# ogulcanaydogan/llm-slo-ebpf-toolkit

Hardware: AMD Instinct MI355X
Metric: fault-replay attribution throughput through the agent's BPF-ring -> GPU path (events/s, node-wide); held-out attribution macro-F1 and agent CPU overhead % reported alongside (higher is better)
Workload: dtype fp64 posteriors / fp32 features (exact-int64 time joins)

## Files before the change

### llm_slo_ebpf_toolkit_amd/ops/csrc/agent_bindings.cpp

```cpp
#include <pybind11/numpy.h>
#include <pybind11/pybind11.h>
#include <pybind11/stl.h>

#include <cstring>
#include <memory>
#include <stdexcept>

#include "engine.h"
#include "exemplars.h"
#include "openreq.h"
#include "slisketch.h"

namespace py = pybind11;
using namespace mislo;

namespace {

template <class T>
py::array_t<T> copy_array(const T* p, std::vector<py::ssize_t> shape) {
  py::array_t<T> a(shape);
  size_t n = 1;
  for (auto s : shape) n *= (size_t)s;
  if (n) std::memcpy(a.mutable_data(), p, n * sizeof(T));
  return a;
// ... 583 lines not shown
      .def("results", &PyExemplarTracker::results)
      .def("step_ms", &PyExemplarTracker::step_ms)
      .def("resident", &PyExemplarTracker::resident)
      .def("sync", &PyExemplarTracker::sync)
      .def("close", &PyExemplarTracker::close);
  py::class_<PyEngine>(m, "WindowEngine")
      .def(py::init<int, int, int, int, int, int, int, double, double, int, int, bool, bool, int, float, double, int,
                    int, int, int, int, bool>(),
           py::arg("device") = 0, py::arg("sig_cap") = 1 << 20, py::arg("span_cap") = 16384, py::arg("group_cap") = 64,
           py::arg("user_cap") = 1 << 18, py::arg("n_buffers") = 3, py::arg("max_ahead") = 3,
           py::arg("window_ms") = 2000.0, py::arg("threshold") = 0.7, py::arg("fanout") = 3, py::arg("group_mode") = 1,
           py::arg("use_graphs") = true, py::arg("device_refit") = true, py::arg("n_dom") = 10,
           py::arg("ttft_slo_ms") = 800.0f, py::arg("halo_ms") = 0.0, py::arg("import_cap") = 0,
           py::arg("xchg_cap") = 0, py::arg("shard_rank") = 0, py::arg("shard_world") = 1,
           py::arg("halo_windows") = 3, py::arg("split_rings") = false)
      .def("register_host", &PyEngine::register_host)
      .def("submit", &PyEngine::submit, py::arg("k"), py::arg("kernel"), py::arg("user"), py::arg("spans"),
           py::arg("n_groups"), py::arg("labels") = py::none(), py::arg("bases") = std::vector<int64_t>{},
           py::arg("with_labels") = true, py::arg("learn") = false, py::arg("user_rec") = 64)
      .def("h2d_done", &PyEngine::h2d_done)
      .def("wait_h2d", &PyEngine::wait_h2d)
      .def("query", &PyEngine::query)
      .def("wait", &PyEngine::wait)
      .def("packet", &PyEngine::packet)
      .def("results", &PyEngine::results)
      .def("window_ms", &PyEngine::window_ms)
      .def("copy_ms", [](PyEngine& p, int64_t k) {
        py::gil_scoped_release nogil;
        return p.eng().copy_ms(k);
      })
      .def("set_model_bytes", &PyEngine::set_model_bytes)
      .def("set_app_model", &PyEngine::set_app_model)
      .def("set_p0", &PyEngine::set_p0)
      .def("set_refit", &PyEngine::set_refit, py::arg("alpha") = 2.0, py::arg("prior_pseudo") = 1.0,
           py::arg("inv_temp") = 1.0, py::arg("min_count") = 0.0, py::arg("cap_dom") = -1, py::arg("ceil") = 1.0)
      .def("refit_now", &PyEngine::refit_now)
      .def("set_device_refit", [](PyEngine& p, bool on) { p.eng().set_device_refit(on); })
      .def("score", &PyEngine::score, py::arg("feat"), py::arg("labels") = py::none(), py::arg("app") = py::none())
      .def("set_pods", &PyEngine::set_pods)
      .def("inject_remote", &PyEngine::inject_remote)
      .def("results_all", &PyEngine::results_all)
      .def("set_join_params", &PyEngine::set_join_params)
      .def("init_comm", &PyEngine::init_comm)
      .def("totals", &PyEngine::totals)
      .def("reset_totals", &PyEngine::reset_totals)
      .def("stats_acc", &PyEngine::stats_acc)
      .def("model_bytes", &PyEngine::model_bytes)
      .def("restore", &PyEngine::restore)
      .def("sync", &PyEngine::sync)
      .def("import_state", &PyEngine::import_state)
      .def("sent_block", &PyEngine::sent_block)
      .def("close", &PyEngine::close)
      .def_property_readonly("buffers", &PyEngine::buffers)
      .def_property_readonly("windows_folded", &PyEngine::folded)
      .def_property_readonly("graphs", &PyEngine::graphs)
      .def_property_readonly("host_issue_us", &PyEngine::host_issue_us)
      .def_property_readonly("host_wait_us", &PyEngine::host_wait_us)
      .def_property_readonly("host_dma_issue_us", &PyEngine::host_dma_issue_us)
      .def_property_readonly("host_launch_us", &PyEngine::host_launch_us)
      .def_property_readonly("host_pre_us", [](PyEngine& p) { return p.eng().host_pre_us(); })
      .def_property_readonly("host_dma_split_us", [](PyEngine& p) { return p.eng().host_dma_split_us(); })
      .def_property_readonly("host_tail_us", [](PyEngine& p) { return p.eng().host_tail_us(); })
      .def_property_readonly("has_comm", &PyEngine::has_comm)
      .def_property_readonly("rank", [](PyEngine& p) { return p.eng().rank(); })
      .def_property_readonly("world", [](PyEngine& p) { return p.eng().world(); })
      .def_property_readonly("staged_bytes", &PyEngine::staged_bytes)
      .def_property_readonly("direct_bytes", &PyEngine::direct_bytes);
}
```

### llm_slo_ebpf_toolkit_amd/ops/csrc/engine.h

```cpp
#pragma once

#include <hip/hip_runtime.h>
#include <rccl/rccl.h>

#include <map>
#include <tuple>
#include <type_traits>
#include <vector>

#include "mislo_launch.h"
#include "mislo_packet.h"

namespace mislo {

constexpr uint32_t kCtxRows = 1u << 24;
constexpr uint32_t kPodRows = 1u << 20;
constexpr uint32_t kTraceIdRows = 1u << 24;
constexpr int kHeadBytes = 64;

struct Seg {
  const void* ptr;
  size_t bytes;
};

struct EngineConfig {
  int device = 0;
  int sig_cap = 1 << 20, span_cap = 16384, group_cap = 64;
  int user_cap = 1 << 18;
  int n_buffers = 3, max_ahead = 3;
  double window_ms = 2000.0, threshold = 0.7;
  int fanout = 3, group_mode = 1;
  bool use_graphs = true;
  bool device_refit = true;
  double alpha = 2.0, prior_pseudo = 1.0;
  double inv_temp = 1.0, min_count = 0.0;
  int cap_dom = -1;
  double lik_ceil = 1.0;
  int n_dom = 10;
  float ttft_slo_ms = 800.0f;
  double halo_ms = 0.0;
  int halo_windows = 3;
  int import_cap = 0;
  int xchg_cap = 0;
  int shard_rank = 0, shard_world = 1;
  bool split_rings = false;
};

template <class Byte>
struct ResultViewT {
  template <class T>
  using P = std::conditional_t<std::is_const_v<Byte>, const T, T>*;
  P<double> post;
  P<double> gconf;
  P<float> feat;
  P<int32_t> pred;
  P<uint32_t> evbits;
  P<uint32_t> sli;
  P<uint32_t> app;
  P<uint32_t> late;
};
using ResultView = ResultViewT<const uint8_t>;

struct ResultLayout {
  size_t G;
  size_t gconf() const { return 16 * G * 8; }
  size_t feat() const { return gconf() + G * 8; }
  size_t pred() const { return feat() + 16 * G * 4; }
  size_t evbits() const { return pred() + G * 4; }
  size_t sli() const { return evbits() + 16 * G * 4; }
  size_t bytes() const { return sli() + 6 * G * 4; }
  template <class Byte>
  ResultViewT<Byte> view(Byte* r) const {
    ResultViewT<Byte> v;
    auto set = [r](auto& p, size_t off) { p = reinterpret_cast<std::remove_reference_t<decltype(p)>>(r + off); };
    set(v.post, 0), set(v.gconf, gconf()), set(v.feat, feat()), set(v.pred, pred()), set(v.evbits, evbits());
    set(v.sli, sli()), set(v.app, sli() + 2 * G * 4), set(v.late, sli() + 4 * G * 4);
    return v;
  }
};

struct WindowInput {
  std::vector<Seg> kernel;
  std::vector<Seg> user;
  int user_rec = 64;
  std::vector<Seg> spans;
  int n_groups = 0;
  const int32_t* labels = nullptr;
  int64_t bases[4] = {0, 0, 0, 0};
};

class WindowEngine {
 public:
  explicit WindowEngine(const EngineConfig& cfg);
  ~WindowEngine();
  WindowEngine(const WindowEngine&) = delete;
  WindowEngine& operator=(const WindowEngine&) = delete;

  const EngineConfig& config() const { return cfg_; }
  int buffers() const { return nb_; }

  bool register_host(const void* ptr, size_t bytes);
  void submit(int64_t k, const WindowInput& in, bool with_labels, bool learn);
  bool h2d_done(int64_t k);
  void wait_h2d(int64_t k);
  bool query(int64_t k);
  void wait(int64_t k);
  const double* packet(int64_t k) const { return bufs_[k % nb_].packet_host; }
  ResultView results(int64_t k) const { return layout().view<const uint8_t>(bufs_[k % nb_].res_host); }
  ResultLayout layout() const { return ResultLayout{(size_t)cfg_.group_cap}; }
  std::pair<float, float> window_ms(int64_t k);
  std::vector<float> copy_ms(int64_t k);

  void set_model_bytes(const void* bytes, size_t n);
  void set_refit(double alpha, double prior_pseudo, double inv_temp, double min_count, int cap_dom = -1,
                 double ceil = 1.0);
  void refit_now();
  void set_device_refit(bool on) { cfg_.device_refit = on; }
  void score_features(const float* feat, int n, const int32_t* labels, double* post, int32_t* pred, double* conf,
                      uint32_t* evbits, uint32_t* confusion, const uint32_t* app_cnt = nullptr);
  void set_app_model(const void* bytes, size_t n);
  void set_p0(const double* p0, size_t n);
  void set_pods(const uint32_t* pods, const uint32_t* svcnode, size_t n);
  void inject_remote(const void* blocks, size_t stride, int world, int me);
  void set_join_params(double window_ms, double threshold, int fanout, int group_mode);
  void init_comm(const ncclUniqueId& id, int rank, int world);
  bool has_comm() const { return comm_ != nullptr; }
  int rank() const { return rank_; }
  int world() const { return world_; }
  const uint8_t* results_all(int64_t k) const { return comm_ ? bufs_[k % nb_].res_all_host : bufs_[k % nb_].res_host; }
  size_t result_bytes() const { return layout().bytes(); }

  void totals(double* out);
  void reset_totals();
  void stats_acc(double* out);
  void restore(const double* stats, const void* model, size_t model_bytes, int64_t folded);
  void model_bytes(void* out);
  void sync();
  std::vector<int64_t> import_state();
  std::vector<uint8_t> sent_block();
  int64_t windows_folded() const { return folded_; }
  size_t staged_bytes() const { return staged_bytes_; }
  size_t direct_bytes() const { return direct_bytes_; }
  size_t graphs() const { return graphs_.size(); }
  double host_issue_us() const { return issue_n_ ? issue_us_ / issue_n_ : 0.0; }
  double host_wait_us() const { return issue_n_ ? wait_us_ / issue_n_ : 0.0; }
  double host_dma_issue_us() const { return issue_n_ ? dma_us_ / issue_n_ : 0.0; }
  double host_launch_us() const { return issue_n_ ? launch_us_ / issue_n_ : 0.0; }
  double host_pre_us() const { return issue_n_ ? pre_us_ / issue_n_ : 0.0; }
  double host_tail_us() const { return issue_n_ ? tail_us_ / issue_n_ : 0.0; }

 private:
  int rec_shard_rank() const { return cfg_.split_rings ? 0 : cfg_.shard_rank; }
  int rec_shard_world() const { return cfg_.split_rings ? 1 : cfg_.shard_world; }
  struct Buf;
  enum class Stage : int { Window, Records, Join, XchgSpans, XchgHead, Front, Back };
  static constexpr int kStageSlots = 8;
  void alloc();
// ... 29 lines not shown
  EngineConfig cfg_;
  int nb_, max_ahead_;
  size_t off_kern_ = 0, off_user_ = 0, off_span_ = 0, in_bytes_ = 0;
  size_t kern_bytes() const { return (size_t)kRecStride * (((size_t)cfg_.sig_cap + kBatchSlots - 1) / kBatchSlots); }
  std::vector<std::pair<const uint8_t*, size_t>> registered_;
  size_t staged_bytes_ = 0, direct_bytes_ = 0;
  uint32_t *pod_sn_ = nullptr, *pod_host_ = nullptr;
  unsigned long long* trace_hash_ = nullptr;
  AppModel* app_dev_ = nullptr;
  int n_rows_ = 0;
  int gens_ = 1;
  int slots_ = 1;
  unsigned long long* tmax_ = nullptr;
  KeyTs* g_keys_ = nullptr;
  uint32_t *remote_n_ = nullptr, *sel_cnt_ = nullptr, *sel_off_ = nullptr;
  unsigned long long* sel_mask_ = nullptr;
  int sel_stride_ = 0;
  uint8_t *xsend_ = nullptr, *xrecv_ = nullptr;
  size_t xstride_ = 0, xrecv_bytes_ = 0;
  int nblk_imp_ = 0;
  bool spin_ = false;
  std::vector<uint8_t> inject_;
  size_t inject_stride_ = 0;
  int inject_world_ = 0, inject_me_ = 0;
  int rank_ = 0, world_ = 1;
  hipStream_t side_ = nullptr;
  hipStream_t front_ = nullptr;
  bool overlap_ = false;
  struct BufSet {
    GenMeta* gen;
    int* rows;
    uint32_t *ring_state, *hist, *status, *confusion, *cnt, *gcnt;
    unsigned long long *misc, *dbg, *top3, *gsum;
    double *stats, *stats_count;
    SpanRec* s_rec;
    PartCodes* s_part;
    uint32_t *s_items, *s_part_base, *probe_work;
    PreSpan* s_pre;
  };
  std::vector<BufSet> sets_;
  struct Buf {
    int b;
    uint8_t* in;
    uint8_t* head_host;
    uint8_t* staging;
    double *packet_dev, *packet_host;
    uint8_t *res_dev, *res_host;
    uint8_t *res_all_dev, *res_all_host;
    ResultViewT<uint8_t> res;
    SigRec* imp;
    uint32_t* remote_n;
    const BufSet* set;
    const GenMeta* gen_prev;
    hipEvent_t h2d_done, h2d_part, head_done, front_done, compute_done, comm_done, xchg_done;
    hipEvent_t t_start, t_copy_end, t_comp0, t_comp1, t_end;
    const int* counts() const { return reinterpret_cast<const int*>(in); }
  };
  std::vector<Buf> bufs_;
  hipEvent_t ev_fork_ = nullptr, ev_sigbase_ = nullptr, ev_spans_ = nullptr;
  bool branch_ = false;
  bool xspan_ = false;
  bool exchange() const { return comm_ && cfg_.xchg_cap > 0 && cfg_.import_cap > 0; }
  JoinParams jp_{};
  int nblk_sig_ = 1, nblk_span_ = 1;
  hipStream_t copy_ = nullptr, copy2_ = nullptr, compute_ = nullptr, comm_stream_ = nullptr;
  ncclComm_t comm_ = nullptr;
  ncclComm_t xcomm_ = nullptr;
  uint32_t* ctx_tab_ = nullptr;
  double *totals_ = nullptr, *stats_acc_ = nullptr, *p0_ = nullptr;
  uint8_t* model_dev_ = nullptr;
  std::vector<uint8_t*> model_host_;
  int model_slot_ = 0;
  uint8_t* g_status_ = nullptr;
  PartCodes* g_part_ = nullptr;
  uint32_t *g_part_blk_ = nullptr, *g_part_off_ = nullptr, *g_part_tot_ = nullptr, *g_part_base_ = nullptr,
           *g_items_ = nullptr;
  SigRec* g_rec_ = nullptr;
  uint32_t *s_part_blk_ = nullptr, *s_part_off_ = nullptr, *s_part_tot_ = nullptr;
  float *attrs_ = nullptr, *conf_ = nullptr, *kernel_ms_ = nullptr;
  std::map<std::tuple<int, int, bool, bool>, hipGraphExec_t> graphs_;
  std::vector<bool> warm_;
  std::vector<hipGraph_t> graph_defs_;
  int64_t submitted_ = 0, folded_ = 0;
  double issue_us_ = 0, wait_us_ = 0, dma_us_ = 0, launch_us_ = 0, pre_us_ = 0, tail_us_ = 0;
  double split_us_[4] = {0, 0, 0, 0};

 public:
  std::vector<double> host_dma_split_us() const {
    std::vector<double> v;
    for (double x : split_us_) v.push_back(issue_n_ ? x / issue_n_ : 0.0);
    return v;
  }

 private:
  int64_t issue_n_ = 0;
};

void engine_set_tables(const Tables& t);

}
```

### llm_slo_ebpf_toolkit_amd/ops/csrc/engine.hip

```cpp
#include "engine.h"
#include "mislo_packet_kernels.h"

#include <algorithm>
#include <chrono>
#include <cstdlib>
#include <cmath>
#include <cstring>
#include <stdexcept>
#include <string>

namespace mislo {

namespace {

#define HIPCHECK(x)                                                                                  \
  do {                                                                                               \
    hipError_t _e = (x);                                                                             \
    if (_e != hipSuccess) throw std::runtime_error(std::string("HIP error: ") + hipGetErrorString(_e) + \
                                                   " at " #x);                                       \
  } while (0)

#define NCCLCHECK(x)                                                                                        \
  do {                                                                                                      \
    ncclResult_t _r = (x);                                                                                  \
    if (_r != ncclSuccess) throw std::runtime_error(std::string("RCCL error: ") + ncclGetErrorString(_r) + \
                                                    " at " #x);                                             \
  } while (0)

__global__ void k_accumulate(const double* __restrict__ packet, double* __restrict__ totals, int n,
                             double* __restrict__ host) {
  const int i = blockIdx.x * blockDim.x + threadIdx.x;
  if (i < n) {
    const double v = packet[i];
    totals[i] += v;
    host[i] = v;
  }
}

__global__ __launch_bounds__(256) void k_window_end(const uint32_t* hist, const uint32_t* status,
                                                    const unsigned long long* misc, const unsigned long long* dbg,
                                                    const uint32_t* confusion, const double* stats, const double* count,
                                                    const uint32_t* ring, double* __restrict__ packet,
                                                    double* __restrict__ totals, double* __restrict__ packet_host,
                                                    const uint4* __restrict__ res, uint4* __restrict__ res_host,
                                                    size_t res16) {
  const size_t t = blockIdx.x * (size_t)blockDim.x + threadIdx.x, stride = (size_t)gridDim.x * blockDim.x;
  if (t < (size_t)kPacketLen) {
    const double v = packet_value((int)t, hist, status, misc, dbg, confusion, stats, count, ring);
    packet[t] = v;
    totals[t] += v;
    packet_host[t] = v;
  }
  for (size_t i = t; i < res16; i += stride) res_host[i] = res[i];
}

__global__ void k_to_host(const uint4* __restrict__ src, uint4* __restrict__ dst, size_t n16) {
  for (size_t i = blockIdx.x * (size_t)blockDim.x + threadIdx.x; i < n16; i += (size_t)gridDim.x * blockDim.x)
    dst[i] = src[i];
}

void to_host(const void* src, void* dst, size_t bytes, hipStream_t st) {
  const size_t n16 = (bytes + 15) / 16;
  const int g = (int)std::min<size_t>(64, (n16 + 255) / 256);
  hipLaunchKernelGGL(k_to_host, dim3(g > 0 ? g : 1), dim3(256), 0, st, static_cast<const uint4*>(src),
                     static_cast<uint4*>(dst), n16);
}

constexpr unsigned kEvWait = hipEventDisableTiming | hipEventBlockingSync;

int env_int(const char* name, int unset) {
  const char* v = getenv(name);
  return v ? atoi(v) : unset;
}

struct Lap {
  using clock = std::chrono::steady_clock;
  clock::time_point t = clock::now();
  void operator()(double& acc) {
    const auto n = clock::now();
    acc += std::chrono::duration<double, std::micro>(n - t).count();
    t = n;
  }
};

}

void engine_set_tables(const Tables& t) { set_tables(&t); }

template <class T>
T* WindowEngine::dalloc(size_t n, bool zero) {
  void* p = nullptr;
  HIPCHECK(hipMalloc(&p, n * sizeof(T) + 64));
  own_.dev.push_back(p);
  if (zero) HIPCHECK(hipMemset(p, 0, n * sizeof(T)));
  return static_cast<T*>(p);
}

void* WindowEngine::host_alloc(size_t bytes, unsigned flags) {
  void* h = nullptr;
  HIPCHECK(hipHostMalloc(&h, bytes, flags));
  own_.host.push_back(h);
  return h;
}

void* WindowEngine::host_block(size_t bytes) {
  void* h = host_alloc((bytes + 15) & ~size_t(15), hipHostMallocCoherent | hipHostMallocMapped);
  std::memset(h, 0, bytes);
  return h;
}

hipEvent_t WindowEngine::mk_event(unsigned flags) {
  hipEvent_t e;
  HIPCHECK(hipEventCreateWithFlags(&e, flags));
  own_.events.push_back(e);
  return e;
}

hipStream_t WindowEngine::mk_stream(bool high_priority) {
  hipStream_t s;
  int lo = 0, hi = 0;
  if (high_priority) {
    HIPCHECK(hipDeviceGetStreamPriorityRange(&lo, &hi));
// ... 12 lines not shown
}

WindowEngine::Owner::~Owner() {
  for (hipEvent_t e : events) (void)hipEventDestroy(e);
  for (void* p : host) (void)hipHostFree(p);
  for (void* p : dev) (void)hipFree(p);
  for (hipStream_t s : streams) (void)hipStreamDestroy(s);
}

WindowEngine::WindowEngine(const EngineConfig& cfg) : cfg_(cfg) {
  if (cfg.sig_cap <= 0 || cfg.span_cap <= 0 || cfg.group_cap <= 0 || cfg.group_cap > 4096)
    throw std::invalid_argument("capacities out of range");
  if (cfg.sig_cap >= (1 << 27)) throw std::invalid_argument("sig_cap must be < 2^27 (top-3 key packing)");
  nb_ = std::max(2, cfg.n_buffers);
  max_ahead_ = std::min(nb_, std::max(1, cfg.max_ahead));
  if (cfg.user_cap <= 0 || cfg.user_cap > cfg.sig_cap) throw std::invalid_argument("user_cap must be in [1, sig_cap]");
  if (cfg.import_cap < 0 || cfg.xchg_cap < 0 || cfg.halo_ms < 0) throw std::invalid_argument("negative import sizes");
  if (cfg.halo_windows < 1 || cfg.halo_windows >= kMaxGens)
    throw std::invalid_argument("halo_windows must be in [1, 3] (resident generations)");
  gens_ = cfg.halo_ms > 0 ? 1 + cfg.halo_windows : 1;
  if (2LL * gens_ * ((long long)cfg.sig_cap + cfg.import_cap) >= (1LL << 27))
    throw std::invalid_argument("2 x generations x (sig_cap + import_cap) must be < 2^27 (top-3 key packing)");
  HIPCHECK(hipSetDevice(cfg.device));
  set_join_params(cfg.window_ms, cfg.threshold, cfg.fanout, cfg.group_mode);
  alloc();
}

void WindowEngine::set_join_params(double window_ms, double threshold, int fanout, int group_mode) {
  const int64_t ms = 1000000;
  int64_t outer = (int64_t)llround(window_ms * ms);
  if (outer <= 0) outer = 2000 * ms;
  if (outer >= (1LL << 35)) throw std::invalid_argument("window too large for top-3 key packing (< 34 s)");
  jp_.outer_ns = outer;
  const int64_t tw[4] = {outer, 100 * ms, 250 * ms, 500 * ms};
  for (int k = 0; k < 4; ++k) jp_.win_ns[k] = std::min(outer, tw[k]);
  const float cf[4] = {1.0f, 0.9f, 0.8f, 0.65f};
  for (int k = 0; k < 4; ++k) jp_.conf[k] = cf[k];
  jp_.threshold = threshold > 0 ? (float)threshold : 0.7f;
  if (fanout <= 0) fanout = 3;
  if (fanout > 3) throw std::invalid_argument("GPU join keeps at most 3 candidates per span");
  jp_.fanout = fanout;
  jp_.group_mode = group_mode;
  graphs_.clear();
}

void WindowEngine::alloc() {
  const int64_t S = cfg_.span_cap, G = cfg_.group_cap;
  n_rows_ = cfg_.sig_cap + cfg_.import_cap;
  const int64_t N = n_rows_;
  nblk_sig_ = decode_grid((int)N);
  nblk_span_ = decode_grid((int)S);
  const bool one_stream = env_int("MISLO_ONE_STREAM", 0) == 1;
  compute_ = mk_stream();
  copy_ = one_stream ? compute_ : mk_stream();
  spin_ = env_int("MISLO_SPIN_WAIT", 0) == 1;
  copy2_ = env_int("MISLO_COPY_STREAMS", 0) == 2 && !one_stream ? mk_stream() : copy_;
  overlap_ = env_int("MISLO_WINDOW_OVERLAP", !one_stream) == 1 && !one_stream &&
             !(cfg_.xchg_cap > 0 && cfg_.import_cap > 0);
  if (overlap_) front_ = mk_stream();
  slots_ = gens_ + (overlap_ ? 1 : 0);
  {
    if (env_int("MISLO_SPAN_STREAM", !one_stream && !overlap_) == 1) enable_span_branch();
  }
  comm_stream_ = compute_;
  const size_t head = (kHeadBytes + 4 * (size_t)G + 63) & ~size_t(63);
  off_kern_ = head;
  off_user_ = (off_kern_ + kern_bytes() + 63) & ~size_t(63);
  off_span_ = off_user_ + 64 * (size_t)cfg_.user_cap;
  in_bytes_ = off_span_ + 64 * (size_t)S;
  const ResultLayout lay = layout();
  bufs_.assign(nb_, Buf{});
  for (Buf& buf : bufs_) {
    buf.in = dalloc<uint8_t>(in_bytes_, true);
    buf.head_host = static_cast<uint8_t*>(host_block(head));
    buf.packet_dev = dalloc<double>(kPacketLen, true);
    buf.packet_host = static_cast<double*>(host_block(kPacketLen * sizeof(double)));
    for (hipEvent_t* e : {&buf.h2d_done, &buf.h2d_part, &buf.head_done, &buf.compute_done, &buf.comm_done,
                          &buf.front_done, &buf.xchg_done})
      *e = mk_event(kEvWait);
    for (hipEvent_t* e : {&buf.t_start, &buf.t_copy_end, &buf.t_comp0, &buf.t_comp1, &buf.t_end})
      *e = mk_event(hipEventDefault);
    buf.res_host = static_cast<uint8_t*>(host_block(lay.bytes()));
    buf.res_dev = dalloc<uint8_t>(lay.bytes(), true);
    buf.res = lay.view(buf.res_dev);
    buf.imp = cfg_.import_cap ? dalloc<SigRec>(cfg_.import_cap) : nullptr;
  }
  warm_.assign(kStageSlots * nb_, false);
  pod_sn_ = dalloc<uint32_t>(kPodRows, true);
  pod_host_ = static_cast<uint32_t*>(host_alloc(kPodRows * 4, hipHostMallocDefault));
  std::memset(pod_host_, 0, kPodRows * 4);
  trace_hash_ = dalloc<unsigned long long>(kTraceIdRows, true);
  tmax_ = dalloc<unsigned long long>(1, true);
  remote_n_ = dalloc<uint32_t>(nb_, true);
  for (int i = 0; i < (overlap_ ? nb_ : 1); ++i) {
    BufSet s{};
    s.rows = dalloc<int>(16, true);
    s.ring_state = dalloc<uint32_t>(kRsLen);
    s.gen = dalloc<GenMeta>(1);
    GenMeta g{};
    g.cur = (uint32_t)slots_ - 1;
    for (int a = 0; a < kMaxGens; ++a) g.cut[a] = INT64_MAX;
    HIPCHECK(hipMemcpy(s.gen, &g, sizeof(g), hipMemcpyHostToDevice));
    s.s_part = dalloc<PartCodes>(S);
    s.s_part_base = dalloc<uint32_t>(kKeyTypes * kParts + 1);
    s.s_items = dalloc<uint32_t>(kKeyTypes * S);
    s.s_pre = dalloc<PreSpan>((size_t)kKeyTypes * S);
    s.s_rec = dalloc<SpanRec>(S);
    s.probe_work = dalloc<uint32_t>(kProbeWorkLen, true);
    s.top3 = dalloc<unsigned long long>(3 * S);
    s.cnt = dalloc<uint32_t>(S);
    s.gsum = dalloc<unsigned long long>((size_t)kGroupStripes * G * kSlots);
    s.gcnt = dalloc<uint32_t>((size_t)kGroupStripes * G * kSlots);
    s.hist = dalloc<uint32_t>(kSlots * kBuckets);
    s.status = dalloc<uint32_t>(kSlots * 3);
    s.misc = dalloc<unsigned long long>(kPacketMisc);
    s.dbg = dalloc<unsigned long long>(kPacketDbg);
    s.confusion = dalloc<uint32_t>(kMaxDomains * kMaxDomains);
    s.stats = dalloc<double>(32 * 32);
    s.stats_count = dalloc<double>(kMaxDomains);
    sets_.push_back(s);
  }
  for (int b = 0; b < nb_; ++b) {
    bufs_[b].b = b;
    bufs_[b].set = &sets_[overlap_ ? b : 0];
    bufs_[b].gen_prev = sets_[overlap_ ? (b + nb_ - 1) % nb_ : 0].gen;
    bufs_[b].remote_n = remote_n_ + b;
  }
  sel_cnt_ = dalloc<uint32_t>(1024);
  sel_off_ = dalloc<uint32_t>(1024);
  xstride_ = sizeof(XRec) * (1 + (size_t)cfg_.xchg_cap);
  if (cfg_.xchg_cap) {
    xsend_ = dalloc<uint8_t>(xstride_, true);
    if (env_int("MISLO_SEL_TWO_PASS", 0) != 1) {
// ... 41 lines not shown
  if (branch_) return;
  side_ = mk_stream(env_int("MISLO_SPAN_STREAM_PRIO", 0) == 1);
  for (hipEvent_t* e : {&ev_fork_, &ev_sigbase_, &ev_spans_}) *e = mk_event(hipEventDisableTiming);
  xspan_ = env_int("MISLO_XCHG_SPAN_SIDE", 1) != 0;
  branch_ = true;
}

SignalCols WindowEngine::sig_cols(const Buf& buf) const {
  return SignalCols{g_rec_, g_status_, g_part_, g_items_, g_keys_, g_part_base_, buf.set->gen, (int64_t)n_rows_, gens_,
                    slots_};
}
SpanCols WindowEngine::span_cols(const Buf& buf) const { return SpanCols{buf.set->s_rec, buf.set->s_part}; }

bool WindowEngine::register_host(const void* ptr, size_t bytes) {
  if (!ptr || !bytes) return false;
  if (registered(ptr, bytes)) return true;
  if (hipHostRegister(const_cast<void*>(ptr), bytes, hipHostRegisterDefault) != hipSuccess) {
    (void)hipGetLastError();
    return false;
  }
  registered_.emplace_back(static_cast<const uint8_t*>(ptr), bytes);
  return true;
}

bool WindowEngine::registered(const void* p, size_t n) const {
  const uint8_t* q = static_cast<const uint8_t*>(p);
  for (const auto& r : registered_)
    if (q >= r.first && q + n <= r.first + r.second) return true;
  return false;
}

size_t WindowEngine::dma(const std::vector<Seg>& segs, uint8_t* dst, size_t cap, uint8_t*& staging, size_t& st_off,
                         hipStream_t st) {
  size_t off = 0;
  for (const Seg& s : segs) {
    if (!s.bytes) continue;
    if (off + s.bytes > cap) throw std::invalid_argument("window input exceeds the engine's capacity");
    const void* src = s.ptr;
    if (!registered(s.ptr, s.bytes)) {
      if (!staging) staging = static_cast<uint8_t*>(host_alloc(in_bytes_ - off_kern_, hipHostMallocDefault));
      std::memcpy(staging + st_off, s.ptr, s.bytes);
      src = staging + st_off;
      st_off += s.bytes;
      staged_bytes_ += s.bytes;
    } else {
      direct_bytes_ += s.bytes;
    }
    HIPCHECK(hipMemcpyAsync(dst + off, src, s.bytes, hipMemcpyHostToDevice, st));
    off += s.bytes;
  }
  return off;
}

bool WindowEngine::h2d_done(int64_t k) {
  for (hipEvent_t ev : {bufs_[k % nb_].h2d_done, bufs_[k % nb_].h2d_part}) {
    const hipError_t e = hipEventQuery(ev);
    if (e == hipErrorNotReady) return false;
    HIPCHECK(e);
  }
  return true;
}

void WindowEngine::wait_h2d(int64_t k) {
  HIPCHECK(hipEventSynchronize(bufs_[k % nb_].h2d_done));
  HIPCHECK(hipEventSynchronize(bufs_[k % nb_].h2d_part));
}

void WindowEngine::run_begin(const Buf& buf, hipStream_t st) {
  const BufSet& s = *buf.set;
  const int S = cfg_.span_cap, G = cfg_.group_cap;
  FillList fl{};
  auto add = [&](void* p, size_t bytes, uint32_t v) { fl.seg[fl.count++] = FillSeg{(uint32_t*)p, (uint32_t)(bytes / 4), v}; };
  add(s.hist, kSlots * kBuckets * 4, 0);
  add(s.status, kSlots * 3 * 4, 0);
  add(s.misc, kPacketMisc * 8, 0);
  add(s.dbg, kPacketDbg * 8, 0);
  add(s.confusion, kMaxDomains * kMaxDomains * 4, 0);
  add(s.stats, 32 * 32 * 8, 0);
  add(s.stats_count, kMaxDomains * 8, 0);
  add(s.top3, 3 * (size_t)S * 8, 0xFFFFFFFFu);
  add(s.cnt, (size_t)S * 4, 0);
  add(s.gsum, (size_t)kGroupStripes * G * kSlots * 8, 0);
  add(s.gcnt, (size_t)kGroupStripes * G * kSlots * 4, 0);
  add(buf.res.sli, (size_t)G * 6 * 4, 0);
  launch_window_begin(fl, s.gen, buf.gen_prev, tmax_, gens_, slots_, (long long)llround(cfg_.halo_ms * 1e6),
                      s.ring_state, buf.remote_n, buf.counts(), n_rows_, s.rows, st);
}

void WindowEngine::run_part1(const Buf& buf, hipStream_t st, bool xchg) {
  const BufSet& s = *buf.set;
  const int* counts = buf.counts();
  const int N = n_rows_;
  if (!(xchg && xspan_)) run_begin(buf, st);
  if (branch_ && !xchg) run_span_branch(buf, st);
  const TraceIds tt{trace_hash_, kTraceIdRows};
  launch_ring_defs(buf.in + off_kern_, counts, cfg_.sig_cap, ctx_tab_, kCtxRows, pod_sn_, kPodRows, tt, s.ring_state,
                   st);
  const bool fused_sel = xchg && sel_mask_;
  launch_decode_window(buf.in + off_kern_, buf.in + off_user_, counts, s.rows, N, buf.imp, ctx_tab_, (int)kCtxRows, tt,
                       s.ring_state, tmax_, pod_sn_, kPodRows, sig_cols(buf), s.hist, s.status, g_part_blk_, s.misc, st,
                       0, 0, 0, rec_shard_rank(), rec_shard_world(), fused_sel ? sel_cnt_ : nullptr,
                       fused_sel ? sel_mask_ : nullptr, sel_stride_);
  if (fused_sel)
    launch_select_masked(sig_cols(buf), s.rows, N, sel_cnt_, sel_off_, sel_mask_, sel_stride_,
                         reinterpret_cast<XRec*>(xsend_ + sizeof(XRec)), reinterpret_cast<uint32_t*>(xsend_),
                         (uint32_t)cfg_.xchg_cap, st, s.dbg + kDbgXchgDropped);
  else if (xchg)
    launch_select(sig_cols(buf), s.rows, counts, N, sel_cnt_, sel_off_, reinterpret_cast<XRec*>(xsend_ + sizeof(XRec)),
                  reinterpret_cast<uint32_t*>(xsend_), (uint32_t)cfg_.xchg_cap, st, s.dbg + kDbgXchgDropped);
}

void WindowEngine::run_join_front(const Buf& buf, hipStream_t st, bool xchg) {
  const BufSet& s = *buf.set;
  const int N = n_rows_;
  if (xchg) {
    const TraceIds tt{trace_hash_, kTraceIdRows};
    launch_decode_window(buf.in + off_kern_, buf.in + off_user_, buf.counts(), s.rows, N, buf.imp, ctx_tab_,
                         (int)kCtxRows, tt, s.ring_state, tmax_, pod_sn_, kPodRows, sig_cols(buf), s.hist, s.status,
// ... 88 lines not shown
                                  : std::make_tuple(slot, n_groups, with_labels, learn);
  auto it = graphs_.find(key);
  if (it == graphs_.end() && !warm_[slot]) {
    run();
    warm_[slot] = true;
    return;
  }
  if (it == graphs_.end()) {
    hipGraph_t g;
    HIPCHECK(hipStreamBeginCapture(cs, hipStreamCaptureModeThreadLocal));
    run();
    HIPCHECK(hipStreamEndCapture(cs, &g));
    hipGraphExec_t ex;
    HIPCHECK(hipGraphInstantiate(&ex, g, nullptr, nullptr, 0));
    graph_defs_.push_back(g);
    it = graphs_.emplace(key, ex).first;
  }
  HIPCHECK(hipGraphLaunch(it->second, cs));
}

void WindowEngine::merge_remote(const Buf& buf, const uint8_t* blocks, size_t stride, int world, int me,
                                hipStream_t st) {
  launch_remote_merge(blocks, stride, world, me, buf.imp, buf.remote_n, (uint32_t)cfg_.import_cap, cfg_.xchg_cap, st,
                      buf.set->dbg + kDbgXchgDropped);
  launch_window_rows(buf.counts(), buf.remote_n, n_rows_, buf.set->rows, buf.set->gen, st);
}

void WindowEngine::refit(const double* add) {
  launch_refit_nb(stats_acc_, add, p0_, cfg_.alpha, cfg_.prior_pseudo, cfg_.n_dom,
                  reinterpret_cast<PosteriorModel*>(model_dev_), compute_, cfg_.inv_temp, cfg_.min_count,
                  p0_ + kSlots * 16, cfg_.cap_dom, cfg_.lik_ceil);
}

void WindowEngine::submit(int64_t k, const WindowInput& in, bool with_labels, bool learn) {
  Lap whole;
  if (k != submitted_) throw std::invalid_argument("windows must be submitted in order");
  const int n_groups = in.n_groups;
  if (n_groups < 0 || n_groups > cfg_.group_cap) throw std::invalid_argument("n_groups exceeds group capacity");
  size_t kb = 0, ub = 0, sb = 0;
  for (const Seg& s : in.kernel) kb += s.bytes;
  for (const Seg& s : in.user) ub += s.bytes;
  for (const Seg& s : in.spans) sb += s.bytes;
  if (in.user_rec != 64 && in.user_rec != 32 && in.user_rec != 24 && in.user_rec != 16)
    throw std::invalid_argument("user records are 64, 32, 24 or 16 bytes");
  if (kb % kRecStride || ub % in.user_rec || sb % 64) throw std::invalid_argument("segments must hold whole records");
  const size_t n_k = kb / kRecStride * kBatchSlots, n_u = ub / in.user_rec, n_s = sb / 64;
  if (n_k + n_u > (size_t)cfg_.sig_cap || n_u > (size_t)cfg_.user_cap || n_s > (size_t)cfg_.span_cap)
    throw std::invalid_argument("window exceeds the engine's capacity (events / user records / spans)");
  Buf& buf = bufs_[k % nb_];
  Lap phase;
  if (k >= max_ahead_) HIPCHECK(hipEventSynchronize(bufs_[(k - max_ahead_) % nb_].compute_done));
  if (k >= nb_) {
    HIPCHECK(hipEventSynchronize(buf.h2d_done));
    HIPCHECK(hipEventSynchronize(buf.h2d_part));
    HIPCHECK(hipEventSynchronize(buf.head_done));
  }
  phase(wait_us_);
  int32_t* c = reinterpret_cast<int32_t*>(buf.head_host);
  std::memset(c, 0, kHeadBytes);
  c[0] = (int32_t)(n_k + n_u);
  c[1] = (int32_t)n_s;
  c[2] = n_groups;
  c[4] = (int32_t)(uint32_t)(uint64_t)in.bases[0];
  c[5] = (int32_t)(uint32_t)((uint64_t)in.bases[0] >> 32);
  c[6] = in.user_rec;
  c[7] = 64;
  for (int q = 1; q < 4; ++q) {
    c[8 + 2 * (q - 1)] = (int32_t)(uint32_t)(uint64_t)in.bases[q];
    c[9 + 2 * (q - 1)] = (int32_t)(uint32_t)((uint64_t)in.bases[q] >> 32);
  }
  c[15] = (int32_t)n_k;
  int32_t* lab = reinterpret_cast<int32_t*>(buf.head_host + kHeadBytes);
  for (int g = 0; g < cfg_.group_cap; ++g) lab[g] = (in.labels && g < n_groups) ? in.labels[g] : -1;
  HIPCHECK(hipStreamWaitEvent(copy_, buf.compute_done, 0));
  HIPCHECK(hipStreamWaitEvent(copy2_, buf.compute_done, 0));
  HIPCHECK(hipEventRecord(buf.t_start, copy_));
  size_t st_off = 0;
  Lap part;
  dma(in.kernel, buf.in + off_kern_, kern_bytes(), buf.staging, st_off, copy_);
  part(split_us_[0]);
  part(split_us_[1]);
  dma(in.user, buf.in + off_user_, 64 * (size_t)cfg_.user_cap, buf.staging, st_off, copy2_);
  part(split_us_[2]);
  dma(in.spans, buf.in + off_span_, 64 * (size_t)cfg_.span_cap, buf.staging, st_off, copy2_);
  part(split_us_[3]);
  HIPCHECK(hipEventRecord(buf.h2d_part, copy2_));
  HIPCHECK(hipEventRecord(buf.h2d_done, copy_));
  HIPCHECK(hipEventRecord(buf.t_copy_end, copy2_));
  phase(dma_us_);
  hipStream_t fs = overlap_ ? front_ : compute_;
  HIPCHECK(hipStreamWaitEvent(fs, buf.h2d_done, 0));
  HIPCHECK(hipStreamWaitEvent(fs, buf.h2d_part, 0));
  if (overlap_ && k >= 2) HIPCHECK(hipStreamWaitEvent(fs, bufs_[(k - 2) % nb_].compute_done, 0));
  HIPCHECK(hipStreamWaitEvent(compute_, buf.comm_done, 0));
  const bool injected = !inject_.empty();
  if (injected) {
    HIPCHECK(hipMemcpyAsync(xrecv_, inject_.data(), inject_.size(), hipMemcpyHostToDevice, compute_));
    HIPCHECK(hipStreamSynchronize(compute_));
  }
  HIPCHECK(hipEventRecord(buf.t_comp0, fs));
  to_host(buf.head_host, buf.in, off_kern_, fs);
  HIPCHECK(hipEventRecord(buf.head_done, fs));
  if (cfg_.device_refit && k >= nb_) {
    refit(buf.packet_dev + kStatsOff);
    ++folded_;
  }
  const bool xchg = exchange() || injected;
  phase(pre_us_);
  if (overlap_) {
    if (xchg) throw std::logic_error("the exchange path does not run with overlapped windows");
    launch_part(Stage::Front, buf, n_groups, with_labels, learn);
    HIPCHECK(hipEventRecord(buf.front_done, front_));
    HIPCHECK(hipStreamWaitEvent(compute_, buf.front_done, 0));
    launch_part(Stage::Back, buf, n_groups, with_labels, learn);
  } else if (!xchg) {
    launch_part(Stage::Window, buf, n_groups, with_labels, learn);
  } else {
    if (xspan_) {
      launch_part(Stage::XchgHead, buf, n_groups, with_labels, learn);
      HIPCHECK(hipEventRecord(ev_fork_, compute_));
      HIPCHECK(hipStreamWaitEvent(side_, ev_fork_, 0));
      launch_part(Stage::XchgSpans, buf, n_groups, with_labels, learn);
      HIPCHECK(hipEventRecord(ev_spans_, side_));
    }
    launch_part(Stage::Records, buf, n_groups, with_labels, learn);
    if (injected) {
      merge_remote(buf, xrecv_, inject_stride_, inject_world_, inject_me_, compute_);
      inject_.clear();
    } else if (xcomm_) {
      NCCLCHECK(ncclAllGather(xsend_, xrecv_, xstride_, ncclUint8, xcomm_, compute_));
      merge_remote(buf, xrecv_, xstride_, world_, rank_, compute_);
    } else {
      HIPCHECK(hipEventRecord(buf.xchg_done, compute_));
      HIPCHECK(hipStreamWaitEvent(comm_stream_, buf.xchg_done, 0));
      NCCLCHECK(ncclAllGather(xsend_, xrecv_, xstride_, ncclUint8, comm_, comm_stream_));
      merge_remote(buf, xrecv_, xstride_, world_, rank_, comm_stream_);
      HIPCHECK(hipEventRecord(buf.xchg_done, comm_stream_));
      HIPCHECK(hipStreamWaitEvent(compute_, buf.xchg_done, 0));
    }
    if (xspan_) HIPCHECK(hipStreamWaitEvent(compute_, ev_spans_, 0));
    launch_part(Stage::Join, buf, n_groups, with_labels, learn);
  }
  phase(launch_us_);
  const size_t res_bytes = result_bytes();
  if (comm_) to_host(buf.res_dev, buf.res_host, res_bytes, compute_);
  HIPCHECK(hipEventRecord(buf.t_comp1, compute_));
  HIPCHECK(hipEventRecord(buf.compute_done, compute_));
  HIPCHECK(hipStreamWaitEvent(comm_stream_, buf.compute_done, 0));
  if (comm_) {
    NCCLCHECK(ncclGroupStart());
    NCCLCHECK(ncclAllReduce(buf.packet_dev, buf.packet_dev, kPacketLen - kPacketRing, ncclFloat64, ncclSum, comm_,
                            comm_stream_));
    NCCLCHECK(ncclAllGather(buf.res_dev, buf.res_all_dev, res_bytes, ncclUint8, comm_, comm_stream_));
    NCCLCHECK(ncclGroupEnd());
    to_host(buf.res_all_dev, buf.res_all_host, res_bytes * world_, comm_stream_);
    hipLaunchKernelGGL(k_accumulate, dim3((kPacketLen + 255) / 256), dim3(256), 0, comm_stream_, buf.packet_dev,
                       totals_, kPacketLen, buf.packet_host);
  }
  HIPCHECK(hipEventRecord(buf.t_end, comm_stream_));
  HIPCHECK(hipEventRecord(buf.comm_done, comm_stream_));
  ++submitted_;
  phase(tail_us_);
  whole(issue_us_);
  ++issue_n_;
}

bool WindowEngine::query(int64_t k) {
  const hipError_t e = hipEventQuery(bufs_[k % nb_].comm_done);
  if (e == hipSuccess) return true;
  if (e == hipErrorNotReady) return false;
  HIPCHECK(e);
  return false;
}

void WindowEngine::wait(int64_t k) {
  if (spin_) {
    while (!query(k)) {
    }
    return;
  }
  HIPCHECK(hipEventSynchronize(bufs_[k % nb_].comm_done));
}

std::vector<float> WindowEngine::copy_ms(int64_t k) {
  const Buf& buf = bufs_[k % nb_];
  float dur = 0.f, gap = -1.f;
  HIPCHECK(hipEventSynchronize(buf.t_copy_end));
  HIPCHECK(hipEventElapsedTime(&dur, buf.t_start, buf.t_copy_end));
  if (k >= 1 && nb_ > 1) HIPCHECK(hipEventElapsedTime(&gap, bufs_[(k - 1) % nb_].t_copy_end, buf.t_start));
  return {dur, gap};
}

std::pair<float, float> WindowEngine::window_ms(int64_t k) {
  const Buf& buf = bufs_[k % nb_];
  float total = 0.f, comp = 0.f;
  HIPCHECK(hipEventSynchronize(buf.t_end));
  HIPCHECK(hipEventElapsedTime(&total, buf.t_start, buf.t_end));
  HIPCHECK(hipEventElapsedTime(&comp, buf.t_comp0, buf.t_comp1));
  return {total, comp};
}

void WindowEngine::set_model_bytes(const void* bytes, size_t n) {
  if (n != sizeof(PosteriorModel)) throw std::invalid_argument("model image must be POSTERIOR_MODEL_BYTES bytes");
  uint8_t* h = model_host_[model_slot_++ % model_host_.size()];
  std::memcpy(h, bytes, n);
  HIPCHECK(hipMemcpyAsync(model_dev_, h, n, hipMemcpyHostToDevice, compute_));
}

void WindowEngine::set_app_model(const void* bytes, size_t n) {
  if (n != sizeof(AppModel)) throw std::invalid_argument("application model must be APP_MODEL_BYTES bytes");
  uint8_t* h = model_host_[model_slot_++ % model_host_.size()];
  static_assert(sizeof(AppModel) <= sizeof(PosteriorModel), "the staging slots fit the application model");
  std::memcpy(h, bytes, n);
  HIPCHECK(hipMemcpyAsync(app_dev_, h, n, hipMemcpyHostToDevice, compute_));
}

void WindowEngine::set_p0(const double* p0, size_t n) {
  if (n != (size_t)kSlots * 16 && n != 2 * (size_t)kSlots * 16) throw std::invalid_argument("p0 must be f64[256] or [512]");
  HIPCHECK(hipMemset(p0_ + kSlots * 16, 0, kSlots * 16 * sizeof(double)));
  HIPCHECK(hipMemcpy(p0_, p0, n * sizeof(double), hipMemcpyHostToDevice));
}

void WindowEngine::set_refit(double alpha, double prior_pseudo, double inv_temp, double min_count, int cap_dom,
                             double ceil) {
  if (!(alpha > 0.0) || !(prior_pseudo >= 0.0) || !(inv_temp > 0.0) || !(min_count >= 0.0) || cap_dom >= cfg_.n_dom ||
      !(ceil > 0.0 && ceil <= 1.0))
    throw std::invalid_argument("refit parameters");
  cfg_.lik_ceil = ceil;
  cfg_.cap_dom = cap_dom < 0 ? -1 : cap_dom;
  cfg_.alpha = alpha;
  cfg_.prior_pseudo = prior_pseudo;
  cfg_.inv_temp = inv_temp;
  cfg_.min_count = min_count;
}

void WindowEngine::refit_now() { refit(nullptr); }

void WindowEngine::score_features(const float* feat, int n, const int32_t* labels, double* post, int32_t* pred,
                                  double* conf, uint32_t* evbits, uint32_t* confusion, const uint32_t* app_cnt) {
  if (n < 0) throw std::invalid_argument("n");
  sync();
  if (n == 0) return;
// ... 34 lines not shown
  std::vector<uint8_t> out(xsend_ ? xstride_ : 0);
  if (xsend_) HIPCHECK(hipMemcpy(out.data(), xsend_, xstride_, hipMemcpyDeviceToHost));
  return out;
}

std::vector<int64_t> WindowEngine::import_state() {
  sync();
  int rows[2];
  unsigned long long tmax = 0;
  GenMeta g{};
  std::vector<uint32_t> r(nb_);
  const BufSet& s = *bufs_[submitted_ ? (submitted_ - 1) % nb_ : 0].set;
  HIPCHECK(hipMemcpy(rows, s.rows, sizeof(rows), hipMemcpyDeviceToHost));
  HIPCHECK(hipMemcpy(&tmax, tmax_, 8, hipMemcpyDeviceToHost));
  HIPCHECK(hipMemcpy(&g, s.gen, sizeof(g), hipMemcpyDeviceToHost));
  HIPCHECK(hipMemcpy(r.data(), remote_n_, 4 * nb_, hipMemcpyDeviceToHost));
  std::vector<int64_t> out{rows[0], rows[1], (int64_t)tmax, gens_, g.cur, g.filled};
  for (int a = 0; a < kMaxGens; ++a) out.push_back(g.cut[a]);
  for (int a = 0; a < kMaxGens; ++a) out.push_back(a < gens_ ? g.n_rows[(g.cur + slots_ - a) % slots_] : 0);
  for (int b = 0; b < nb_; ++b) out.push_back(r[b]);
  return out;
}

void WindowEngine::inject_remote(const void* blocks, size_t stride, int world, int me) {
  if (!cfg_.import_cap || !cfg_.xchg_cap) throw std::logic_error("inject_remote needs import_cap and xchg_cap > 0");
  if (world < 1 || me < 0 || me >= world || stride < sizeof(XRec)) throw std::invalid_argument("bad exchange blocks");
  const uint8_t* h = static_cast<const uint8_t*>(blocks);
  for (int r = 0; r < world; ++r) {
    uint32_t c;
    std::memcpy(&c, h + (size_t)r * stride, 4);
    if ((size_t)c * sizeof(XRec) + sizeof(XRec) > stride) throw std::invalid_argument("block row count exceeds stride");
    if (r != me && c > (uint32_t)cfg_.xchg_cap) throw std::invalid_argument("block holds more rows than xchg_cap");
  }
  if (stride * world > xrecv_bytes_) {
    sync();
    own_.free_dev(xrecv_);
    xrecv_ = dalloc<uint8_t>(stride * world);
    xrecv_bytes_ = stride * world;
  }
  inject_.assign(h, h + stride * world);
  inject_stride_ = stride;
  inject_world_ = world;
  inject_me_ = me;
}

void WindowEngine::init_comm(const ncclUniqueId& id, int rank, int world) {
  if (comm_) throw std::logic_error("communicator already initialised");
  if (world < 1 || rank < 0 || rank >= world) throw std::invalid_argument("communicator rank / world");
  if (submitted_) throw std::logic_error("init_comm before the first window");
  HIPCHECK(hipSetDevice(cfg_.device));
  if (overlap_) {
    HIPCHECK(hipStreamSynchronize(front_));
    overlap_ = false;
    if (!getenv("MISLO_SPAN_STREAM")) enable_span_branch();
  }
  NCCLCHECK(ncclCommInitRank(&comm_, world, id, rank));
  {
    comm_stream_ = mk_stream(env_int("MISLO_COMM_STREAM_PRIO", 1) != 0);
  }
  rank_ = rank;
  world_ = world;
  for (Buf& buf : bufs_) {
    buf.res_all_dev = dalloc<uint8_t>(result_bytes() * world);
    buf.res_all_host = static_cast<uint8_t*>(host_block(result_bytes() * world));
  }
  if (cfg_.xchg_cap) {
    if (world > 8) throw std::invalid_argument("the exchange is sized for <= 8 GPUs per node");
    own_.free_dev(xrecv_);
    xrecv_bytes_ = xstride_ * world;
    xrecv_ = dalloc<uint8_t>(xrecv_bytes_, true);
    const char* xv = getenv("MISLO_XCHG_STREAM");
    int split = (xv && std::strcmp(xv, "compute") == 0) ? 1 : 0;
    int* d_split = dalloc<int>(1);
    HIPCHECK(hipMemcpy(d_split, &split, sizeof(int), hipMemcpyHostToDevice));
    NCCLCHECK(ncclBroadcast(d_split, d_split, 1, ncclInt32, 0, comm_, comm_stream_));
    HIPCHECK(hipStreamSynchronize(comm_stream_));
    HIPCHECK(hipMemcpy(&split, d_split, sizeof(int), hipMemcpyDeviceToHost));
    own_.free_dev(d_split);
    if (split) NCCLCHECK(ncclCommSplit(comm_, 0, rank, &xcomm_, nullptr));
  }
}

void WindowEngine::totals(double* out) {
  sync();
  HIPCHECK(hipMemcpy(out, totals_, kPacketLen * sizeof(double), hipMemcpyDeviceToHost));
}

void WindowEngine::reset_totals() {
  sync();
  HIPCHECK(hipMemset(totals_, 0, kPacketLen * sizeof(double)));
}

void WindowEngine::stats_acc(double* out) {
  sync();
  HIPCHECK(hipMemcpy(out, stats_acc_, kStatsLen * sizeof(double), hipMemcpyDeviceToHost));
}

void WindowEngine::restore(const double* stats, const void* model, size_t n, int64_t folded) {
  if (n && n != sizeof(PosteriorModel)) throw std::invalid_argument("model image must be POSTERIOR_MODEL_BYTES bytes");
  sync();
  HIPCHECK(hipMemcpy(stats_acc_, stats, kStatsLen * sizeof(double), hipMemcpyHostToDevice));
  if (n) {
    HIPCHECK(hipMemcpy(model_dev_, model, n, hipMemcpyHostToDevice));
  } else {
    refit(nullptr);
    HIPCHECK(hipStreamSynchronize(compute_));
  }
  folded_ = folded;
}

void WindowEngine::model_bytes(void* out) {
  sync();
  HIPCHECK(hipMemcpy(out, model_dev_, sizeof(PosteriorModel), hipMemcpyDeviceToHost));
}

void WindowEngine::sync() {
  HIPCHECK(hipStreamSynchronize(copy_));
  if (copy2_ != copy_) HIPCHECK(hipStreamSynchronize(copy2_));
  if (front_) HIPCHECK(hipStreamSynchronize(front_));
  HIPCHECK(hipStreamSynchronize(compute_));
  HIPCHECK(hipStreamSynchronize(comm_stream_));
}

}
```

Before: 2.441 billion.

## Alternate whole-window H2D copies across two copy lanes instead of splitting streams

Replaces the old per-window split of the kernel/user/span uploads across two copy streams with per-window copy lanes. Consecutive windows alternate between two streams, so one window's full upload can overlap the next. It also drops the copy streams' wait on compute_done and removes the extra h2d_part and t_copy_end events. A monotone CopiedUpTo tracker preserves in-order completion semantics for h2d_done and wait_h2d. The risks are extra stream contention and the ordering subtleties introduced by removing the copy-stream wait.

```diff
diff --git a/llm_slo_ebpf_toolkit_amd/ops/csrc/agent_bindings.cpp b/llm_slo_ebpf_toolkit_amd/ops/csrc/agent_bindings.cpp
--- a/llm_slo_ebpf_toolkit_amd/ops/csrc/agent_bindings.cpp
+++ b/llm_slo_ebpf_toolkit_amd/ops/csrc/agent_bindings.cpp
@@ -659,6 +659,7 @@
       .def("sent_block", &PyEngine::sent_block)
       .def("close", &PyEngine::close)
       .def_property_readonly("buffers", &PyEngine::buffers)
+      .def_property_readonly("copy_lanes", [](PyEngine& p) { return p.eng().copy_lanes(); })
       .def_property_readonly("windows_folded", &PyEngine::folded)
       .def_property_readonly("graphs", &PyEngine::graphs)
       .def_property_readonly("host_issue_us", &PyEngine::host_issue_us)
diff --git a/llm_slo_ebpf_toolkit_amd/ops/csrc/copylanes.h b/llm_slo_ebpf_toolkit_amd/ops/csrc/copylanes.h
--- /dev/null
+++ b/llm_slo_ebpf_toolkit_amd/ops/csrc/copylanes.h
@@ -0,0 +1,36 @@
+#pragma once
+
+#include <cstdint>
+
+namespace mislo {
+
+constexpr int kMaxCopyLanes = 2;
+
+inline int copy_lane(int64_t k, int lanes) { return lanes > 1 ? (int)(k % lanes) : 0; }
+
+inline int copy_consults(int64_t k, int lanes, int64_t out[kMaxCopyLanes]) {
+  int n = 0;
+  for (int i = 0; i < (lanes > 1 ? lanes : 1) && k - i >= 0; ++i) out[n++] = k - i;
+  return n;
+}
+
+struct CopiedUpTo {
+  int64_t n = 0;
+
+  void reused(int64_t k, int nb) {
+    if (k - nb + 1 > n) n = k - nb + 1;
+  }
+
+  template <class Ready>
+  bool done(int64_t k, int lanes, Ready&& ready) {
+    if (k < n) return true;
+    int64_t w[kMaxCopyLanes];
+    const int c = copy_consults(k, lanes, w);
+    for (int i = 0; i < c; ++i)
+      if (w[i] >= n && !ready(w[i])) return false;
+    n = k + 1;
+    return true;
+  }
+};
+
+}
diff --git a/llm_slo_ebpf_toolkit_amd/ops/csrc/engine.h b/llm_slo_ebpf_toolkit_amd/ops/csrc/engine.h
--- a/llm_slo_ebpf_toolkit_amd/ops/csrc/engine.h
+++ b/llm_slo_ebpf_toolkit_amd/ops/csrc/engine.h
@@ -8,6 +8,7 @@
 #include <type_traits>
 #include <vector>
 
+#include "copylanes.h"
 #include "mislo_launch.h"
 #include "mislo_packet.h"
 
@@ -103,6 +104,7 @@
   void submit(int64_t k, const WindowInput& in, bool with_labels, bool learn);
   bool h2d_done(int64_t k);
   void wait_h2d(int64_t k);
+  int copy_lanes() const { return lanes_; }
   bool query(int64_t k);
   void wait(int64_t k);
   const double* packet(int64_t k) const { return bufs_[k % nb_].packet_host; }
@@ -238,8 +240,8 @@
     uint32_t* remote_n;
     const BufSet* set;
     const GenMeta* gen_prev;
-    hipEvent_t h2d_done, h2d_part, head_done, front_done, compute_done, comm_done, xchg_done;
-    hipEvent_t t_start, t_copy_end, t_comp0, t_comp1, t_end;
+    hipEvent_t h2d_done, head_done, front_done, compute_done, comm_done, xchg_done;
+    hipEvent_t t_start, t_comp0, t_comp1, t_end;
     const int* counts() const { return reinterpret_cast<const int*>(in); }
   };
   std::vector<Buf> bufs_;
@@ -249,7 +251,11 @@
   bool exchange() const { return comm_ && cfg_.xchg_cap > 0 && cfg_.import_cap > 0; }
   JoinParams jp_{};
   int nblk_sig_ = 1, nblk_span_ = 1;
-  hipStream_t copy_ = nullptr, copy2_ = nullptr, compute_ = nullptr, comm_stream_ = nullptr;
+  hipStream_t copy_[kMaxCopyLanes] = {nullptr, nullptr};
+  int lanes_ = 1;
+  CopiedUpTo copied_;
+  bool copied_ready(int64_t w, bool block);
+  hipStream_t compute_ = nullptr, comm_stream_ = nullptr;
   ncclComm_t comm_ = nullptr;
   ncclComm_t xcomm_ = nullptr;
   uint32_t* ctx_tab_ = nullptr;
diff --git a/llm_slo_ebpf_toolkit_amd/ops/csrc/engine.hip b/llm_slo_ebpf_toolkit_amd/ops/csrc/engine.hip
--- a/llm_slo_ebpf_toolkit_amd/ops/csrc/engine.hip
+++ b/llm_slo_ebpf_toolkit_amd/ops/csrc/engine.hip
@@ -67,7 +67,6 @@
 }
 
 constexpr unsigned kEvWait = hipEventDisableTiming | hipEventBlockingSync;
-
 int env_int(const char* name, int unset) {
   const char* v = getenv(name);
   return v ? atoi(v) : unset;
@@ -186,12 +185,13 @@
   nblk_span_ = decode_grid((int)S);
   const bool one_stream = env_int("MISLO_ONE_STREAM", 0) == 1;
   compute_ = mk_stream();
-  copy_ = one_stream ? compute_ : mk_stream();
+  copy_[0] = one_stream ? compute_ : mk_stream();
   spin_ = env_int("MISLO_SPIN_WAIT", 0) == 1;
-  copy2_ = env_int("MISLO_COPY_STREAMS", 0) == 2 && !one_stream ? mk_stream() : copy_;
   overlap_ = env_int("MISLO_WINDOW_OVERLAP", !one_stream) == 1 && !one_stream &&
              !(cfg_.xchg_cap > 0 && cfg_.import_cap > 0);
   if (overlap_) front_ = mk_stream();
+  lanes_ = overlap_ && env_int("MISLO_COPY_LANES", nb_ >= 4 ? 2 : 1) == 2 ? 2 : 1;
+  copy_[1] = lanes_ == 2 ? mk_stream(env_int("MISLO_COPY_LANE_PRIO", 1) != 0) : copy_[0];
   slots_ = gens_ + (overlap_ ? 1 : 0);
   {
     if (env_int("MISLO_SPAN_STREAM", !one_stream && !overlap_) == 1) enable_span_branch();
@@ -209,10 +209,10 @@
     buf.head_host = static_cast<uint8_t*>(host_block(head));
     buf.packet_dev = dalloc<double>(kPacketLen, true);
     buf.packet_host = static_cast<double*>(host_block(kPacketLen * sizeof(double)));
-    for (hipEvent_t* e : {&buf.h2d_done, &buf.h2d_part, &buf.head_done, &buf.compute_done, &buf.comm_done,
-                          &buf.front_done, &buf.xchg_done})
+    for (hipEvent_t* e : {&buf.head_done, &buf.compute_done, &buf.comm_done, &buf.front_done, &buf.xchg_done})
       *e = mk_event(kEvWait);
-    for (hipEvent_t* e : {&buf.t_start, &buf.t_copy_end, &buf.t_comp0, &buf.t_comp1, &buf.t_end})
+    buf.h2d_done = mk_event(hipEventBlockingSync);
+    for (hipEvent_t* e : {&buf.t_start, &buf.t_comp0, &buf.t_comp1, &buf.t_end})
       *e = mk_event(hipEventDefault);
     buf.res_host = static_cast<uint8_t*>(host_block(lay.bytes()));
     buf.res_dev = dalloc<uint8_t>(lay.bytes(), true);
@@ -360,18 +360,26 @@
   return off;
 }
 
+bool WindowEngine::copied_ready(int64_t w, bool block) {
+  const hipEvent_t ev = bufs_[w % nb_].h2d_done;
+  if (block) {
+    HIPCHECK(hipEventSynchronize(ev));
+    return true;
+  }
+  const hipError_t e = hipEventQuery(ev);
+  if (e == hipErrorNotReady) return false;
+  HIPCHECK(e);
+  return true;
+}
+
 bool WindowEngine::h2d_done(int64_t k) {
-  for (hipEvent_t ev : {bufs_[k % nb_].h2d_done, bufs_[k % nb_].h2d_part}) {
-    const hipError_t e = hipEventQuery(ev);
-    if (e == hipErrorNotReady) return false;
-    HIPCHECK(e);
-  }
-  return true;
+  if (k < 0 || k >= submitted_) return false;
+  return copied_.done(k, lanes_, [this](int64_t w) { return copied_ready(w, false); });
 }
 
 void WindowEngine::wait_h2d(int64_t k) {
-  HIPCHECK(hipEventSynchronize(bufs_[k % nb_].h2d_done));
-  HIPCHECK(hipEventSynchronize(bufs_[k % nb_].h2d_part));
+  if (k < 0 || k >= submitted_) throw std::invalid_argument("wait_h2d: the window has not been submitted");
+  copied_.done(k, lanes_, [this](int64_t w) { return copied_ready(w, true); });
 }
 
 void WindowEngine::run_begin(const Buf& buf, hipStream_t st) {
@@ -566,7 +574,7 @@
   if (k >= max_ahead_) HIPCHECK(hipEventSynchronize(bufs_[(k - max_ahead_) % nb_].compute_done));
   if (k >= nb_) {
     HIPCHECK(hipEventSynchronize(buf.h2d_done));
-    HIPCHECK(hipEventSynchronize(buf.h2d_part));
+    copied_.reused(k, nb_);
     HIPCHECK(hipEventSynchronize(buf.head_done));
   }
   phase(wait_us_);
@@ -586,25 +594,21 @@
   c[15] = (int32_t)n_k;
   int32_t* lab = reinterpret_cast<int32_t*>(buf.head_host + kHeadBytes);
   for (int g = 0; g < cfg_.group_cap; ++g) lab[g] = (in.labels && g < n_groups) ? in.labels[g] : -1;
-  HIPCHECK(hipStreamWaitEvent(copy_, buf.compute_done, 0));
-  HIPCHECK(hipStreamWaitEvent(copy2_, buf.compute_done, 0));
-  HIPCHECK(hipEventRecord(buf.t_start, copy_));
+  const hipStream_t cs = copy_[copy_lane(k, lanes_)];
+  HIPCHECK(hipEventRecord(buf.t_start, cs));
   size_t st_off = 0;
   Lap part;
-  dma(in.kernel, buf.in + off_kern_, kern_bytes(), buf.staging, st_off, copy_);
+  dma(in.kernel, buf.in + off_kern_, kern_bytes(), buf.staging, st_off, cs);
   part(split_us_[0]);
   part(split_us_[1]);
-  dma(in.user, buf.in + off_user_, 64 * (size_t)cfg_.user_cap, buf.staging, st_off, copy2_);
+  dma(in.user, buf.in + off_user_, 64 * (size_t)cfg_.user_cap, buf.staging, st_off, cs);
   part(split_us_[2]);
-  dma(in.spans, buf.in + off_span_, 64 * (size_t)cfg_.span_cap, buf.staging, st_off, copy2_);
+  dma(in.spans, buf.in + off_span_, 64 * (size_t)cfg_.span_cap, buf.staging, st_off, cs);
   part(split_us_[3]);
-  HIPCHECK(hipEventRecord(buf.h2d_part, copy2_));
-  HIPCHECK(hipEventRecord(buf.h2d_done, copy_));
-  HIPCHECK(hipEventRecord(buf.t_copy_end, copy2_));
+  HIPCHECK(hipEventRecord(buf.h2d_done, cs));
   phase(dma_us_);
   hipStream_t fs = overlap_ ? front_ : compute_;
   HIPCHECK(hipStreamWaitEvent(fs, buf.h2d_done, 0));
-  HIPCHECK(hipStreamWaitEvent(fs, buf.h2d_part, 0));
   if (overlap_ && k >= 2) HIPCHECK(hipStreamWaitEvent(fs, bufs_[(k - 2) % nb_].compute_done, 0));
   HIPCHECK(hipStreamWaitEvent(compute_, buf.comm_done, 0));
   const bool injected = !inject_.empty();
@@ -699,9 +703,9 @@
 std::vector<float> WindowEngine::copy_ms(int64_t k) {
   const Buf& buf = bufs_[k % nb_];
   float dur = 0.f, gap = -1.f;
-  HIPCHECK(hipEventSynchronize(buf.t_copy_end));
-  HIPCHECK(hipEventElapsedTime(&dur, buf.t_start, buf.t_copy_end));
-  if (k >= 1 && nb_ > 1) HIPCHECK(hipEventElapsedTime(&gap, bufs_[(k - 1) % nb_].t_copy_end, buf.t_start));
+  HIPCHECK(hipEventSynchronize(buf.h2d_done));
+  HIPCHECK(hipEventElapsedTime(&dur, buf.t_start, buf.h2d_done));
+  if (k >= 1 && nb_ > 1) HIPCHECK(hipEventElapsedTime(&gap, bufs_[(k - 1) % nb_].h2d_done, buf.t_start));
   return {dur, gap};
 }
 
@@ -842,6 +846,7 @@
   if (overlap_) {
     HIPCHECK(hipStreamSynchronize(front_));
     overlap_ = false;
+    lanes_ = 1;
     if (!getenv("MISLO_SPAN_STREAM")) enable_span_branch();
   }
   NCCLCHECK(ncclCommInitRank(&comm_, world, id, rank));
@@ -905,8 +910,8 @@
 }
 
 void WindowEngine::sync() {
-  HIPCHECK(hipStreamSynchronize(copy_));
-  if (copy2_ != copy_) HIPCHECK(hipStreamSynchronize(copy2_));
+  HIPCHECK(hipStreamSynchronize(copy_[0]));
+  if (copy_[1] != copy_[0]) HIPCHECK(hipStreamSynchronize(copy_[1]));
   if (front_) HIPCHECK(hipStreamSynchronize(front_));
   HIPCHECK(hipStreamSynchronize(compute_));
   HIPCHECK(hipStreamSynchronize(comm_stream_));
```

Measured after the change: 2.524 billion, median of 6. +3.4%, better.
